# thu-ml/zhusuan

Hardware: NVIDIA H100
Metric: leapfrog-steps*chains/sec (higher is better)
Workload: dtype f32

## Files before the change

zhusuan_b200/csrc/hmc_dense_res.cu:

```cuda
#include "hmc_dense_epilogue.cuh"

namespace {

struct ResEpi {
  const __half* __restrict__ hi_cur; const __half* __restrict__ lo_cur;
  __half* __restrict__ hi_nxt; __half* __restrict__ lo_nxt;
  const __half* __restrict__ hi_cur_s; const __half* __restrict__ lo_cur_s;
  __half* __restrict__ hi_nxt_s; __half* __restrict__ lo_nxt_s;
  const float* __restrict__ p_in; float* __restrict__ p_out;
  float* __restrict__ lp_part; float* __restrict__ k_part;
  int64_t chains; int D;
  float sq, inv_sq, acc_scale;
  float rescale;
};

template <int MODE, int NEXT, int DC, bool SPARE>
__device__ __forceinline__ void epilogue_planes(const ResEpi& a, uint32_t trow, int n, bool n_ok,
                                                int64_t c0, int64_t part_row, int lane, float s2,
                                                float eps_over_m_sq, float inv_m, float b_n,
                                                float mu_n, float& qmax) {
  constexpr int NCOL = BN;
  const uint32_t D = DC ? (uint32_t)DC : (uint32_t)a.D;
  const int64_t chains = a.chains;
  const bool warp_n_ok = __all_sync(0xffffffffu, n_ok);
  const bool fast_tile = warp_n_ok && (c0 + NCOL <= chains);
  const int64_t off_t = c0 * (int64_t)D + n;
  const float* __restrict__ pin0 = a.p_in + off_t;
  float* __restrict__ po0 = a.p_out + off_t;
  const unsigned short* __restrict__ hc0 =
      reinterpret_cast<const unsigned short*>(a.hi_cur) + off_t;
  const unsigned short* __restrict__ lc0 =
      reinterpret_cast<const unsigned short*>(a.lo_cur) + off_t;
  __half* __restrict__ hn0 = NEXT ? a.hi_nxt + off_t : nullptr;
  __half* __restrict__ ln0 = NEXT ? a.lo_nxt + off_t : nullptr;
  __half* __restrict__ hs0 = SPARE ? a.hi_nxt_s + off_t : nullptr;
  __half* __restrict__ ls0 = SPARE ? a.lo_nxt_s + off_t : nullptr;

  auto element = [&](float acc, float p, uint32_t hl, float& pn, float& lpv, float& kv,
                     float& Qn) {
    const float Q = __half2float(__ushort_as_half((unsigned short)(hl & 0xFFFFu))) +
                    __half2float(__ushort_as_half((unsigned short)(hl >> 16)));
    const float g = b_n - a.acc_scale * acc;
    pn = fmaf(s2, g, p);
    if (MODE >= 1) lpv = (Q * a.inv_sq - mu_n) * g;
    if (MODE >= 2) kv = pn * pn * inv_m;
    if (NEXT) Qn = fmaf(eps_over_m_sq, pn, Q);
  };

  if (fast_tile) {
    auto load = [&](float* pe, uint32_t* he, int c) {
      const size_t cb = (size_t)c * D;
#pragma unroll
      for (int j = 0; j < 16; ++j) {
        pe[j] = __ldcg(pin0 + cb + (uint32_t)j * D);
        const uint32_t h = __ldcg(hc0 + cb + (uint32_t)j * D);
        const uint32_t l = __ldcg(lc0 + cb + (uint32_t)j * D);
        he[j] = h | (l << 16);
      }
    };
    float ss_a = 0.f, ss_b = 0.f;
    auto compute = [&](const uint32_t* v, const float* pe, const uint32_t* he, int c, float& ss) {
      const size_t cb = (size_t)c * D;
      float lpv[MODE >= 1 ? 16 : 1], kv[MODE >= 2 ? 16 : 1];
#pragma unroll
      for (int j = 0; j < 16; j += 2) {
        float pn[2], lp1[2] = {0.f, 0.f}, k1[2] = {0.f, 0.f}, Qn[2] = {0.f, 0.f};
#pragma unroll
        for (int t = 0; t < 2; ++t) {
          element(__uint_as_float(v[j + t]), pe[j + t], he[j + t], pn[t], lp1[t], k1[t], Qn[t]);
          po0[cb + (uint32_t)(j + t) * D] = pn[t];
          if (MODE >= 1) lpv[j + t] = lp1[t];
          if (MODE >= 2) kv[j + t] = k1[t];
          if (NEXT && !SPARE) ss = fmaf(Qn[t], Qn[t], ss);
          if (SPARE) qmax = fmaxf(qmax, fabsf(Qn[t]));
        }
        if (NEXT) {
          const __half2 h2 = __floats2half2_rn(Qn[0], Qn[1]);
          const float2 hf = __half22float2(h2);
          const __half2 l2 = __floats2half2_rn(Qn[0] - hf.x, Qn[1] - hf.y);
          hn0[cb + (uint32_t)j * D] = __low2half(h2);
          hn0[cb + (uint32_t)(j + 1) * D] = __high2half(h2);
          ln0[cb + (uint32_t)j * D] = __low2half(l2);
          ln0[cb + (uint32_t)(j + 1) * D] = __high2half(l2);
        }
        if (SPARE) {
          const float x0 = Qn[0] * a.rescale, x1 = Qn[1] * a.rescale;
          const __half2 h2 = __floats2half2_rn(x0, x1);
          const float2 hf = __half22float2(h2);
          const __half2 l2 = __floats2half2_rn(x0 - hf.x, x1 - hf.y);
          hs0[cb + (uint32_t)j * D] = __low2half(h2);
          hs0[cb + (uint32_t)(j + 1) * D] = __high2half(h2);
          ls0[cb + (uint32_t)j * D] = __low2half(l2);
          ls0[cb + (uint32_t)(j + 1) * D] = __high2half(l2);
        }
      }
      if (MODE >= 1) {
        const float sum = warp_transpose_sum16(lpv, lane);
        if (lane < 16) a.lp_part[part_row + c0 + c + lane] = sum;
      }
      if (MODE >= 2) {
        const float sum = warp_transpose_sum16(kv, lane);
        if (lane < 16) a.k_part[part_row + c0 + c + lane] = sum;
      }
    };
    float pa[16], pb[16];
    uint32_t ha[16], hb[16], va[16], vb[16];
    load(pa, ha, 0);
#pragma unroll 1
    for (int c = 0; c < NCOL; c += 32) {
      load(pb, hb, c + 16);
      acc_ld16(trow + 4u * (uint32_t)c, va);
      compute(va, pa, ha, c, ss_a);
      if (c + 32 < NCOL) load(pa, ha, c + 32);
      acc_ld16(trow + 4u * (uint32_t)(c + 16), vb);
      compute(vb, pb, hb, c + 16, ss_b);
    }
    if (NEXT && !SPARE) {
      const float norm = sqrtf(ss_a + ss_b) * (1.f + 0x1p-10f);
      qmax = fmaxf(qmax, norm == norm ? norm : INFINITY);
    }
  } else {
#pragma unroll 1
    for (int c = 0; c < NCOL; c += 16) {
      uint32_t v[16];
      acc_ld16(trow + 4u * (uint32_t)c, v);
      const int64_t cbase = c0 + c;
      if (cbase < chains) {
        const size_t cb = (size_t)c * D;
        float lpv[MODE >= 1 ? 16 : 1], kv[MODE >= 2 ? 16 : 1];
#pragma unroll
        for (int j = 0; j < 16; ++j) {
          const bool ok = n_ok && cbase + j < chains;
          float p = 0.f;
          uint32_t hl = 0u;
          if (ok) {
            p = __ldcg(pin0 + cb + (uint32_t)j * D);
            hl = (uint32_t)__ldcg(hc0 + cb + (uint32_t)j * D) |
                 ((uint32_t)__ldcg(lc0 + cb + (uint32_t)j * D) << 16);
          }
          float pn, lp1 = 0.f, k1 = 0.f, Qn = 0.f;
          element(__uint_as_float(v[j]), p, hl, pn, lp1, k1, Qn);
          const __half hh = __float2half_rn(Qn);
          const __half ll = __float2half_rn(Qn - __half2float(hh));
          if (NEXT && ok) qmax = fmaxf(qmax, fabsf(Qn));
          if (MODE >= 1) lpv[j] = ok ? lp1 : 0.f;
          if (MODE >= 2) kv[j] = ok ? k1 : 0.f;
          if (ok) {
            po0[cb + (uint32_t)j * D] = pn;
            if (NEXT) {
              hn0[cb + (uint32_t)j * D] = hh;
              ln0[cb + (uint32_t)j * D] = ll;
            }
            if (SPARE) {
              const float x = Qn * a.rescale;
              const __half hs = __float2half_rn(x);
              hs0[cb + (uint32_t)j * D] = hs;
              ls0[cb + (uint32_t)j * D] = __float2half_rn(x - __half2float(hs));
            }
          }
        }
        if (MODE >= 1) {
          const float sum = warp_transpose_sum16(lpv, lane);
          if (lane < 16 && cbase + lane < chains) a.lp_part[part_row + cbase + lane] = sum;
        }
        if (MODE >= 2) {
          const float sum = warp_transpose_sum16(kv, lane);
          if (lane < 16 && cbase + lane < chains) a.k_part[part_row + cbase + lane] = sum;
        }
      }
    }
  }
}


__device__ __forceinline__ int& producer_spare_in() {
  __shared__ int spare_in;
  return spare_in;
}

template <int MODE, int NEXT, int DC, int CX, int CY>
struct ResW {
  static constexpr int KIND = 1, RB = 64, MNA = 0, MNB = 0;
  static constexpr int CLUSTER = CX * CY;
  static constexpr int KE = RB / 2;
  static constexpr uint32_t TX = Cfg<RB>::STAGE;
  CUtensorMap m_phi, m_plo, m_qhi, m_qlo, m_shi, m_slo;
  ResEpi ea;
  const float* bvec; const float* mu; const float* mass; const float* state;
  float* scales;
  float p_scale;
  int n_blk, D_rt, pass;
  struct EpiState { float qmax = 0.f; };

  __device__ __forceinline__ int D() const { return DC ? DC : D_rt; }
  __host__ __device__ __forceinline__ int64_t units() const {
    return ((ea.chains + BN - 1) / BN) * (int64_t)n_blk;
  }
  __device__ __forceinline__ void tile(int64_t u, int& nb, int64_t& cb) const {
    const uint64_t cu = (uint64_t)u / CLUSTER;
    const int r = (int)((uint64_t)u % CLUSTER);
    const uint32_t nbx = (uint32_t)(n_blk / CX);
    nb = (int)(cu % nbx) * CX + r % CX;
    cb = (int64_t)(cu / nbx) * CY + r / CX;
  }
  __device__ __forceinline__ void kb_range(int64_t, int& kb0, int& kb1) const {
    kb0 = 0;
    kb1 = D() / KE;
  }
  __device__ __forceinline__ void prefetch() const {
    tma_prefetch_desc(&m_phi); tma_prefetch_desc(&m_plo);
    tma_prefetch_desc(&m_qhi); tma_prefetch_desc(&m_qlo);
    tma_prefetch_desc(&m_shi); tma_prefetch_desc(&m_slo);
    producer_spare_in() = plane_spare_in(scales, pass);
  }
  __device__ __forceinline__ void load(int64_t u, int kb, uint32_t sa, uint32_t fb) const {
    using C = Cfg<RB>;
    int nb;
    int64_t cb;
    tile(u, nb, cb);
    const int n0 = nb * BM;
    const int c0 = (int)cb * BN;
    const bool s = producer_spare_in() != 0;
    const CUtensorMap* qh = s ? &m_shi : &m_qhi;
    const CUtensorMap* ql = s ? &m_slo : &m_qlo;
    const int r = (int)(u % CLUSTER), rx = r % CX, ry = r / CX;
    if constexpr (CY == 1) {
      tma_load_2d(sa, &m_phi, fb, kb * KE, n0);
      tma_load_2d(sa + C::A_TILE, &m_plo, fb, kb * KE, n0);
    } else {
      constexpr int rows = BM / CY;
      uint16_t mask = 0;
#pragma unroll
      for (int y = 0; y < CY; ++y) mask |= (uint16_t)(1u << (y * CX + rx));
      const uint32_t o = (uint32_t)(ry * rows * RB);
      tma_load_2d_mc(sa + o, &m_phi, fb, kb * KE, n0 + ry * rows, mask);
      tma_load_2d_mc(sa + C::A_TILE + o, &m_plo, fb, kb * KE, n0 + ry * rows, mask);
    }
    if constexpr (CX == 1) {
      tma_load_2d(sa + 2 * C::A_TILE, qh, fb, kb * KE, c0);
      tma_load_2d(sa + 2 * C::A_TILE + C::B_TILE, ql, fb, kb * KE, c0);
    } else {
      constexpr int rows = BN / CX;
      const uint16_t mask = (uint16_t)(((1u << CX) - 1u) << (ry * CX));
      const uint32_t o = (uint32_t)(rx * rows * RB);
      tma_load_2d_mc(sa + 2 * C::A_TILE + o, qh, fb, kb * KE, c0 + rx * rows, mask);
      tma_load_2d_mc(sa + 2 * C::A_TILE + C::B_TILE + o, ql, fb, kb * KE, c0 + rx * rows, mask);
    }
  }
  __device__ __forceinline__ float sq_alt(float eps, float sq) const {
    return next_plane_scale(scales, pass, eps, mul(eps, p_scale), sq);
  }
  __device__ __forceinline__ void epilogue(int64_t u, uint32_t trow, int quarter, int lane,
                                           EpiState& st) const {
    int nb;
    int64_t cb;
    tile(u, nb, cb);
    const int n = nb * BM + quarter * 32 + lane;
    const int64_t c0 = cb * BN;
    const bool n_ok = n < D();
    const float eps = state[ZSB_ST_EPS_USED];
    const float s2 = mul(eps, p_scale);
    const bool spare_in = plane_spare_in(scales, pass);
    const float sq = plane_scale_in(scales, pass);
    const float m_n = n_ok ? mass[n] : 1.f;
    const float eps_over_m_sq = mul(fdiv(eps, m_n), sq);
    const float inv_m = fdiv(1.f, m_n);
    const float b_n = (n_ok && bvec) ? bvec[n] : 0.f;
    const float mu_n = (n_ok && mu) ? mu[n] : 0.f;
    const int64_t part_row = (int64_t)(nb * 4 + quarter) * ea.chains;
    ResEpi a = ea;
    if (spare_in) {
      a.hi_cur = ea.hi_cur_s;
      a.lo_cur = ea.lo_cur_s;
    }
    a.sq = sq;
    a.inv_sq = fdiv(1.f, sq);
    a.acc_scale = 1.f / (scales[3] * sq);
    a.rescale = NEXT ? sq_alt(eps, sq) * a.inv_sq : 1.f;
    if (a.rescale == 1.f)
      epilogue_planes<MODE, NEXT, DC, false>(a, trow, n, n_ok, c0, part_row, lane, s2,
                                             eps_over_m_sq, inv_m, b_n, mu_n, st.qmax);
    else
      epilogue_planes<MODE, NEXT, DC, true>(a, trow, n, n_ok, c0, part_row, lane, s2,
                                            eps_over_m_sq, inv_m, b_n, mu_n, st.qmax);
  }
  __device__ __forceinline__ void epi_finish(EpiState& st, int quarter, int lane) const {
    if (!NEXT) return;
    const float sq = plane_scale_in(scales, pass);
    const float alt = sq_alt(state[ZSB_ST_EPS_USED], sq);
    publish_plane_scale(scales, pass, sq, alt, st.qmax * (1.f / sq),
                        alt != sq && !(st.qmax < kHalfOverflow), quarter, lane);
  }
};

constexpr int RES_CX = 2, RES_CY = 1;

template <int DC, int CX, int CY>
int res_pass(const CUtensorMap& phi, const CUtensorMap& plo, const CUtensorMap& qhi,
             const CUtensorMap& qlo, const CUtensorMap& shi, const CUtensorMap& slo,
             const ResEpi& ea, const float* bvec, const float* mu, const float* mass,
             const float* state, float* scales, int pass, float p_scale, int n_blk, int D,
             int mode, cudaStream_t st) {
  if (mode == 1) {
    const ResW<1, 1, DC, CX, CY> w{phi, plo, qhi, qlo, shi, slo, ea, bvec, mu, mass, state,
                                   scales, p_scale, n_blk, D, pass};
    return tc_launch(w, st, "hmc_dense_resident");
  }
  if (mode == 0) {
    const ResW<0, 1, DC, CX, CY> w{phi, plo, qhi, qlo, shi, slo, ea, bvec, mu, mass, state,
                                   scales, p_scale, n_blk, D, pass};
    return tc_launch(w, st, "hmc_dense_resident");
  }
  const ResW<2, 0, DC, CX, CY> w{phi, plo, qhi, qlo, shi, slo, ea, bvec, mu, mass, state, scales,
                                 p_scale, n_blk, D, pass};
  return tc_launch(w, st, "hmc_dense_resident");
}

template <int DC>
int res_pass(bool cluster, const CUtensorMap& phi, const CUtensorMap& plo, const CUtensorMap& qhi,
             const CUtensorMap& qlo, const CUtensorMap& shi, const CUtensorMap& slo,
             const ResEpi& ea, const float* bvec, const float* mu, const float* mass,
             const float* state, float* scales, int pass, float p_scale, int n_blk, int D,
             int mode, cudaStream_t st) {
// ... 35 lines not shown
          const uint32_t lw[4] = {l[u].x, l[u].y, l[u].z, l[u].w};
          float o[8];
#pragma unroll
          for (int k = 0; k < 4; ++k) {
            const float2 hf = __half22float2(*reinterpret_cast<const __half2*>(&hw[k]));
            const float2 lf = __half22float2(*reinterpret_cast<const __half2*>(&lw[k]));
            o[2 * k] = (hf.x + lf.x) * inv_sq;
            o[2 * k + 1] = (hf.y + lf.y) * inv_sq;
          }
          qr[2 * i] = make_float4(o[0], o[1], o[2], o[3]);
          qr[2 * i + 1] = make_float4(o[4], o[5], o[6], o[7]);
        }
      }
    }
  }
}

}

int zsb_dense_res_h16_launch(void* planes0, void* planes1, void* spare0, void* spare1,
                             const float* p0, float* pw,
                             const void* P_h16, const void* P_l16, float* scales,
                             const float* bvec, const float* mu, const float* mass,
                             const float* state, float* lp0_part, float* lp1_part, float* k_part,
                             int64_t chains, int D, int L, cudaStream_t st) {
  if (D % 64 != 0 || D < 64 || L < 1 || chains <= 0 || chains >= (1LL << 31)) {
    zsb_set_error("dense_res: needs D %% 64 == 0, n_leapfrogs >= 1");
    return ZSB_ERR_INVALID;
  }
  if (planes0 == planes1 || !spare0 || !spare1 || spare0 == spare1) {
    zsb_set_error("dense_res: planes1, spare0 and spare1 must be separate work buffers");
    return ZSB_ERR_INVALID;
  }
  const int n_blk = (D + BM - 1) / BM;
  const int64_t c_blk = (chains + BN - 1) / BN;
  const bool cluster = n_blk % RES_CX == 0 && c_blk % RES_CY == 0;
  const uint32_t p_box = cluster ? BM / RES_CY : BM, q_box = cluster ? BN / RES_CX : BN;
  CUtensorMap phi, plo, qhi[2], qlo[2], shi[2], slo[2];
  int rc;
  constexpr int RB = ResW<0, 1, 0, 1, 1>::RB;
  if ((rc = make_map(&phi, P_h16, (uint64_t)D, (uint64_t)D, p_box, RB, 1))) return rc;
  if ((rc = make_map(&plo, P_l16, (uint64_t)D, (uint64_t)D, p_box, RB, 1))) return rc;
  __half* pl[2] = {reinterpret_cast<__half*>(planes0), reinterpret_cast<__half*>(planes1)};
  __half* sp[2] = {reinterpret_cast<__half*>(spare0), reinterpret_cast<__half*>(spare1)};
  const int64_t plane = chains * (int64_t)D;
  for (int b = 0; b < 2; ++b) {
    if ((rc = make_map(&qhi[b], pl[b], (uint64_t)chains, (uint64_t)D, q_box, RB, 1))) return rc;
    if ((rc = make_map(&qlo[b], pl[b] + plane, (uint64_t)chains, (uint64_t)D, q_box, RB, 1)))
      return rc;
    if ((rc = make_map(&shi[b], sp[b], (uint64_t)chains, (uint64_t)D, q_box, RB, 1))) return rc;
    if ((rc = make_map(&slo[b], sp[b] + plane, (uint64_t)chains, (uint64_t)D, q_box, RB, 1)))
      return rc;
  }
  for (int i = 0; i <= L; ++i) {
    const bool last = i == L;
    const int buf = i & 1;
    const ResEpi ea{pl[buf], pl[buf] + plane, pl[buf ^ 1], pl[buf ^ 1] + plane,
                    sp[buf], sp[buf] + plane, sp[buf ^ 1], sp[buf ^ 1] + plane,
                    i == 0 ? p0 : pw, pw, i == 0 ? lp0_part : lp1_part, k_part, chains, D,
                    1.f, 1.f, 1.f, 1.f};
    const int mode = last ? 2 : (i == 0 ? 1 : 0);
    const float p_scale = (i > 0 && !last) ? 1.f : 0.5f;
    rc = (D == 1024)
             ? res_pass<1024>(cluster, phi, plo, qhi[buf], qlo[buf], shi[buf], slo[buf], ea, bvec,
                              mu, mass, state, scales, i, p_scale, n_blk, D, mode, st)
             : res_pass<0>(cluster, phi, plo, qhi[buf], qlo[buf], shi[buf], slo[buf], ea, bvec, mu,
                           mass, state, scales, i, p_scale, n_blk, D, mode, st);
    if (rc != ZSB_OK) return rc;
  }
  return ZSB_OK;
}

#ifdef ZSB_PASS_PROFILE
// ... 23 lines not shown
```

zhusuan_b200/csrc/tc_common.cuh:

```cuda
#pragma once
#include "common.cuh"
#include <cuda.h>
#include <cuda_fp16.h>

namespace {

constexpr int BM = 128;
constexpr int BN = 128;
constexpr int NUM_EPI_WARPS = 4;
constexpr int PRODUCER_WARP = 4;
constexpr int EPI_WARP0 = 5;
constexpr int NUM_THREADS = 32 * (EPI_WARP0 + NUM_EPI_WARPS);
constexpr int ACC_LD = BN + 4;
constexpr int ACC_BYTES = BM * ACC_LD * 4;
constexpr unsigned long long WAIT_TIMEOUT_NS = 2000000000ULL;

enum PassProfSlot {
  PROF_MMA_TOTAL,
  PROF_MMA_FULL,
  PROF_MMA_TEMPTY,
  PROF_MMA_STORE,
  PROF_PROD_EMPTY,
  PROF_EPI_TFULL,
  PROF_EPI_UNIT,
  PROF_UNITS,
  PASS_PROF_SLOTS
};
constexpr int PASS_PROF_CTAS = 1024;
#ifdef ZSB_PASS_PROFILE
constexpr bool kPassProfile = true;
__device__ unsigned long long g_pass_prof[PASS_PROF_CTAS * PASS_PROF_SLOTS];
#else
constexpr bool kPassProfile = false;
#endif
__device__ __forceinline__ long long prof_clock() {
  if constexpr (kPassProfile) return clock64();
  return 0;
}
__device__ __forceinline__ void prof_add(int slot, long long v) {
#ifdef ZSB_PASS_PROFILE
  if (blockIdx.x < PASS_PROF_CTAS)
    atomicAdd(&g_pass_prof[blockIdx.x * PASS_PROF_SLOTS + slot], (unsigned long long)v);
#endif
}

template <int RB>
struct Cfg {
  static constexpr int A_TILE = BM * RB;
  static constexpr int B_TILE = BN * RB;
  static constexpr int STAGE = 2 * A_TILE + 2 * B_TILE;
  static constexpr int STAGES = RB == 128 ? 2 : 5;
  static constexpr int ALIGN = RB == 128 ? 1024 : 512;
  static constexpr int SMEM = STAGES * STAGE + ACC_BYTES + 128 + ALIGN;
  static_assert(SMEM <= 227 * 1024, "operand ring exceeds shared memory");
};

__device__ __forceinline__ uint32_t smem_u32(const void* p) {
  return (uint32_t)__cvta_generic_to_shared(p);
}
__device__ __forceinline__ void mbar_init(uint32_t bar, uint32_t count) {
  asm volatile("mbarrier.init.shared::cta.b64 [%0], %1;" ::"r"(bar), "r"(count) : "memory");
}
__device__ __forceinline__ void mbar_expect_tx(uint32_t bar, uint32_t bytes) {
  asm volatile("mbarrier.arrive.expect_tx.shared::cta.b64 _, [%0], %1;" ::"r"(bar), "r"(bytes)
               : "memory");
}
__device__ __forceinline__ void mbar_arrive(uint32_t bar) {
  asm volatile("mbarrier.arrive.shared::cta.b64 _, [%0];" ::"r"(bar) : "memory");
}
__device__ __forceinline__ bool mbar_try_wait(uint32_t bar, uint32_t parity) {
  uint32_t ok;
  asm volatile(
      "{\n\t.reg .pred P1;\n\t"
      "mbarrier.try_wait.parity.shared::cta.b64 P1, [%1], %2;\n\t"
      "selp.b32 %0, 1, 0, P1;\n\t}"
      : "=r"(ok)
      : "r"(bar), "r"(parity)
      : "memory");
  return ok != 0;
}
__device__ __forceinline__ unsigned long long global_ns() {
  unsigned long long t;
  asm volatile("mov.u64 %0, %%globaltimer;" : "=l"(t));
  return t;
}
__device__ __forceinline__ void mbar_wait(uint32_t bar, uint32_t parity) {
  if (mbar_try_wait(bar, parity)) return;
// ... 45 lines not shown
    d |= (uint64_t)1 << 62;
  } else {
    d |= (uint64_t)1 << 16;
    d |= (uint64_t)((8 * RB) >> 4) << 32;
    d |= (uint64_t)(RB == 128 ? 1 : 2) << 62;
  }
  return d;
}
__device__ __forceinline__ void wgmma_fence() {
  asm volatile("wgmma.fence.sync.aligned;" ::: "memory");
}
__device__ __forceinline__ void wgmma_commit() {
  asm volatile("wgmma.commit_group.sync.aligned;" ::: "memory");
}
template <int N>
__device__ __forceinline__ void wgmma_wait() {
  asm volatile("wgmma.wait_group.sync.aligned %0;" ::"n"(N) : "memory");
}
__device__ __forceinline__ void wgmma_tf32(float (&d)[64], uint64_t da, uint64_t db) {
  asm volatile(
      "{\n\t.reg .pred p;\n\tsetp.ne.b32 p, 1, 0;\n\t"
      "wgmma.mma_async.sync.aligned.m64n128k8.f32.tf32.tf32 {%0, %1, %2, %3, %4, %5, %6, %7, %8, %9, %10, %11, %12, %13, %14, %15, %16, %17, %18, %19, %20, %21, %22, %23, %24, %25, %26, %27, %28, %29, %30, %31, %32, %33, %34, %35, %36, %37, %38, %39, %40, %41, %42, %43, %44, %45, %46, %47, %48, %49, %50, %51, %52, %53, %54, %55, %56, %57, %58, %59, %60, %61, %62, %63}, %64, %65, p, 1, 1;\n\t}"
      : "+f"(d[0]), "+f"(d[1]), "+f"(d[2]), "+f"(d[3]), "+f"(d[4]), "+f"(d[5]), "+f"(d[6]), "+f"(d[7]), "+f"(d[8]), "+f"(d[9]), "+f"(d[10]), "+f"(d[11]), "+f"(d[12]), "+f"(d[13]), "+f"(d[14]), "+f"(d[15]), "+f"(d[16]), "+f"(d[17]), "+f"(d[18]), "+f"(d[19]), "+f"(d[20]), "+f"(d[21]), "+f"(d[22]), "+f"(d[23]), "+f"(d[24]), "+f"(d[25]), "+f"(d[26]), "+f"(d[27]), "+f"(d[28]), "+f"(d[29]), "+f"(d[30]), "+f"(d[31]), "+f"(d[32]), "+f"(d[33]), "+f"(d[34]), "+f"(d[35]), "+f"(d[36]), "+f"(d[37]), "+f"(d[38]), "+f"(d[39]), "+f"(d[40]), "+f"(d[41]), "+f"(d[42]), "+f"(d[43]), "+f"(d[44]), "+f"(d[45]), "+f"(d[46]), "+f"(d[47]), "+f"(d[48]), "+f"(d[49]), "+f"(d[50]), "+f"(d[51]), "+f"(d[52]), "+f"(d[53]), "+f"(d[54]), "+f"(d[55]), "+f"(d[56]), "+f"(d[57]), "+f"(d[58]), "+f"(d[59]), "+f"(d[60]), "+f"(d[61]), "+f"(d[62]), "+f"(d[63])
      : "l"(da), "l"(db));
}
template <int TA, int TB>
__device__ __forceinline__ void wgmma_f16(float (&d)[64], uint64_t da, uint64_t db) {
  asm volatile(
      "{\n\t.reg .pred p;\n\tsetp.ne.b32 p, 1, 0;\n\t"
      "wgmma.mma_async.sync.aligned.m64n128k16.f32.f16.f16 {%0, %1, %2, %3, %4, %5, %6, %7, %8, %9, %10, %11, %12, %13, %14, %15, %16, %17, %18, %19, %20, %21, %22, %23, %24, %25, %26, %27, %28, %29, %30, %31, %32, %33, %34, %35, %36, %37, %38, %39, %40, %41, %42, %43, %44, %45, %46, %47, %48, %49, %50, %51, %52, %53, %54, %55, %56, %57, %58, %59, %60, %61, %62, %63}, %64, %65, p, 1, 1, %66, %67;\n\t}"
      : "+f"(d[0]), "+f"(d[1]), "+f"(d[2]), "+f"(d[3]), "+f"(d[4]), "+f"(d[5]), "+f"(d[6]), "+f"(d[7]), "+f"(d[8]), "+f"(d[9]), "+f"(d[10]), "+f"(d[11]), "+f"(d[12]), "+f"(d[13]), "+f"(d[14]), "+f"(d[15]), "+f"(d[16]), "+f"(d[17]), "+f"(d[18]), "+f"(d[19]), "+f"(d[20]), "+f"(d[21]), "+f"(d[22]), "+f"(d[23]), "+f"(d[24]), "+f"(d[25]), "+f"(d[26]), "+f"(d[27]), "+f"(d[28]), "+f"(d[29]), "+f"(d[30]), "+f"(d[31]), "+f"(d[32]), "+f"(d[33]), "+f"(d[34]), "+f"(d[35]), "+f"(d[36]), "+f"(d[37]), "+f"(d[38]), "+f"(d[39]), "+f"(d[40]), "+f"(d[41]), "+f"(d[42]), "+f"(d[43]), "+f"(d[44]), "+f"(d[45]), "+f"(d[46]), "+f"(d[47]), "+f"(d[48]), "+f"(d[49]), "+f"(d[50]), "+f"(d[51]), "+f"(d[52]), "+f"(d[53]), "+f"(d[54]), "+f"(d[55]), "+f"(d[56]), "+f"(d[57]), "+f"(d[58]), "+f"(d[59]), "+f"(d[60]), "+f"(d[61]), "+f"(d[62]), "+f"(d[63])
      : "l"(da), "l"(db), "n"(TA), "n"(TB));
}

__device__ __forceinline__ void acc_ld16(uint32_t addr, uint32_t v[16]) {
#pragma unroll
  for (int i = 0; i < 4; ++i)
    asm volatile("ld.shared.v4.b32 {%0, %1, %2, %3}, [%4];"
                 : "=r"(v[4 * i]), "=r"(v[4 * i + 1]), "=r"(v[4 * i + 2]), "=r"(v[4 * i + 3])
                 : "r"(addr + 16u * i));
}

__device__ __forceinline__ float warp_transpose_sum16(float v[16], int lane) {
#pragma unroll
  for (int i = 0; i < 16; ++i) v[i] += __shfl_xor_sync(0xffffffffu, v[i], 16);
#pragma unroll
  for (int o = 8, cnt = 16; o >= 1; o >>= 1, cnt >>= 1) {
    const bool upper = (lane & o) != 0;
#pragma unroll
    for (int i = 0; i < cnt / 2; ++i) {
      const float keep = upper ? v[i + cnt / 2] : v[i];
      const float send = upper ? v[i] : v[i + cnt / 2];
      v[i] = keep + __shfl_xor_sync(0xffffffffu, send, o);
    }
  }
  return v[0];
}

__device__ __forceinline__ float pow2_plane_scale(float m) {
  int e = 0;
  if (m > 0.f) frexpf(m, &e);
  return ldexpf(1.f, 12 - e);
}
__device__ __forceinline__ float finite_absmax(float m, float x) {
  const float a = fabsf(x);
  return (a <= 3.0e38f) ? fmaxf(m, a) : m;
}
__device__ __forceinline__ void store_hilo(__half* p, int64_t lo, float x) {
  const __half h = __float2half_rn(x);
  p[0] = h;
  p[lo] = __float2half_rn(x - __half2float(h));
}
__device__ __forceinline__ void fold_amax(float* scale, float m, int lane) {
  m = warp_max(m);
  if (lane == 0 && m > 0.f) atomicMax(reinterpret_cast<unsigned int*>(scale) + 2, __float_as_uint(m));
}

template <int KIND, int RB, int MNA, int MNB, int ZLO = 0>
__device__ __forceinline__ void mma_kblock(float (&d)[2][64], uint32_t sa) {
  using C = Cfg<RB>;
#pragma unroll
  for (int k = 0; k < RB / 32; ++k) {
    const uint32_t bo = MNB ? (uint32_t)k * 2048u : (uint32_t)k * 32u;
    const uint64_t b_hi = gmma_desc<MNB, RB>(sa + 2 * C::A_TILE + bo);
    const uint64_t b_lo = gmma_desc<MNB, RB>(sa + 2 * C::A_TILE + C::B_TILE + bo);
#pragma unroll
    for (int mh = 0; mh < 2; ++mh) {
      const uint32_t ao = MNA ? (uint32_t)mh * 8192u + (uint32_t)k * 2048u
                              : (uint32_t)(mh * 64 * RB) + (uint32_t)k * 32u;
      const uint64_t a_hi = gmma_desc<MNA, RB>(sa + ao);
      const uint64_t a_lo = gmma_desc<MNA, RB>(sa + C::A_TILE + ao);
      if (KIND == 0) {
        wgmma_tf32(d[mh], a_lo, b_hi);
        wgmma_tf32(d[mh], a_hi, b_lo);
        wgmma_tf32(d[mh], a_hi, b_hi);
      } else {
        if (!(ZLO & 1)) wgmma_f16<MNA, MNB>(d[mh], a_lo, b_hi);
        if (!(ZLO & 2)) wgmma_f16<MNA, MNB>(d[mh], a_hi, b_lo);
        wgmma_f16<MNA, MNB>(d[mh], a_hi, b_hi);
      }
    }
  }
}

template <class W, class = void>
struct ClusterOf {
  static constexpr int value = 1;
};
template <class W>
struct ClusterOf<W, decltype((void)W::CLUSTER)> {
  static constexpr int value = W::CLUSTER;
};

template <class W, class = void>
struct ZloOf {
  static constexpr int value = 0;
};
template <class W>
struct ZloOf<W, decltype((void)W::ZLO)> {
  static constexpr int value = W::ZLO;
};

template <class W>
__global__ void __launch_bounds__(NUM_THREADS, 1) tc_pipeline_kernel(const __grid_constant__ W w) {
  using C = Cfg<W::RB>;
  constexpr int CS = ClusterOf<W>::value;
  extern __shared__ uint8_t smem_raw[];
  const uint32_t smem_base = (smem_u32(smem_raw) + (C::ALIGN - 1)) & ~(uint32_t)(C::ALIGN - 1);
  const uint32_t acc_base = smem_base + C::STAGES * C::STAGE;
  const uint32_t bars = acc_base + ACC_BYTES;
  const uint32_t full_bar = bars;
  const uint32_t empty_bar = bars + 8 * C::STAGES;
  const uint32_t tfull_bar = bars + 16 * C::STAGES;
  const uint32_t tempty_bar = tfull_bar + 8;

  const int warp = __shfl_sync(0xffffffffu, (int)(threadIdx.x >> 5), 0);
  const int lane = threadIdx.x & 31;
  const int64_t n_units = w.units();

  if (threadIdx.x == 0) {
    for (int s = 0; s < C::STAGES; ++s) {
      mbar_init(full_bar + 8 * s, 1);
      mbar_init(empty_bar + 8 * s, CS);
    }
    mbar_init(tfull_bar, 128);
    mbar_init(tempty_bar, 32 * NUM_EPI_WARPS);
    asm volatile("fence.mbarrier_init.release.cluster;" ::: "memory");
  }
  if constexpr (CS > 1)
    cluster_sync();
  else
    __syncthreads();
  auto release = [&](int s) {
    if constexpr (CS > 1) {
#pragma unroll
      for (int r = 0; r < CS; ++r) mbar_arrive_cluster(empty_bar + 8 * s, (uint32_t)r);
    } else {
      mbar_arrive(empty_bar + 8 * s);
    }
  };

  if (warp < 4) {
    const int tid = threadIdx.x;
    float d[2][64];
    int stage = 0;
    uint32_t phase = 0, acc_phase = 0;
    const long long t_begin = prof_clock();
    long long t_full = 0, t_tempty = 0, t_store = 0, units = 0;
    for (int64_t u = blockIdx.x; u < n_units; u += gridDim.x) {
      int kb0, kb1;
      w.kb_range(u, kb0, kb1);
#pragma unroll
      for (int mh = 0; mh < 2; ++mh)
#pragma unroll
        for (int i = 0; i < 64; ++i) d[mh][i] = 0.f;
      int prev = -1;
      for (int kb = kb0; kb < kb1; ++kb) {
        const uint32_t sa = smem_base + stage * C::STAGE;
        const long long t0 = prof_clock();
        mbar_spin(full_bar + 8 * stage, phase);
        t_full += prof_clock() - t0;
        wgmma_fence();
        mma_kblock<W::KIND, W::RB, W::MNA, W::MNB, ZloOf<W>::value>(d, sa);
        wgmma_commit();
        wgmma_wait<1>();
        if (prev >= 0 && tid == 0) release(prev);
        prev = stage;
        if (++stage == C::STAGES) { stage = 0; phase ^= 1; }
      }
      wgmma_wait<0>();
      if (prev >= 0 && tid == 0) release(prev);
      const long long t1 = prof_clock();
      mbar_wait(tempty_bar, acc_phase ^ 1);
      const long long t2 = prof_clock();
      t_tempty += t2 - t1;
      const int row = 16 * (tid >> 5) + ((tid & 31) >> 2);
      const int col = 2 * (tid & 3);
#pragma unroll
      for (int mh = 0; mh < 2; ++mh)
#pragma unroll
        for (int j = 0; j < 16; ++j) {
          const uint32_t a0 = acc_base + (uint32_t)(((64 * mh + row) * ACC_LD + 8 * j + col) * 4);
          asm volatile("st.shared.v2.f32 [%0], {%1, %2};" ::"r"(a0), "f"(d[mh][4 * j]),
                       "f"(d[mh][4 * j + 1]) : "memory");
          asm volatile("st.shared.v2.f32 [%0], {%1, %2};" ::"r"(a0 + 8u * ACC_LD * 4u),
                       "f"(d[mh][4 * j + 2]), "f"(d[mh][4 * j + 3]) : "memory");
        }
      mbar_arrive(tfull_bar);
      acc_phase ^= 1;
      t_store += prof_clock() - t2;
      ++units;
    }
    if (kPassProfile && tid == 0) {
      prof_add(PROF_MMA_TOTAL, prof_clock() - t_begin);
      prof_add(PROF_MMA_FULL, t_full);
      prof_add(PROF_MMA_TEMPTY, t_tempty);
      prof_add(PROF_MMA_STORE, t_store);
      prof_add(PROF_UNITS, units);
    }
  } else if (warp == PRODUCER_WARP) {
    if (lane == 0) {
      w.prefetch();
      int stage = 0;
      uint32_t phase = 0;
      long long t_empty = 0;
      for (int64_t u = blockIdx.x; u < n_units; u += gridDim.x) {
        int kb0, kb1;
        w.kb_range(u, kb0, kb1);
        for (int kb = kb0; kb < kb1; ++kb) {
          const long long t0 = prof_clock();
          mbar_wait(empty_bar + 8 * stage, phase ^ 1);
          t_empty += prof_clock() - t0;
          const uint32_t fb = full_bar + 8 * stage;
          mbar_expect_tx(fb, W::TX);
          w.load(u, kb, smem_base + stage * C::STAGE, fb);
          if (++stage == C::STAGES) { stage = 0; phase ^= 1; }
        }
      }
      if (kPassProfile) prof_add(PROF_PROD_EMPTY, t_empty);
    }
  } else {
    const int quarter = warp - EPI_WARP0;
    const uint32_t trow = acc_base + (uint32_t)((quarter * 32 + lane) * ACC_LD * 4);
    typename W::EpiState st;
    uint32_t acc_phase = 0;
    long long t_tfull = 0, t_unit = 0;
    for (int64_t u = blockIdx.x; u < n_units; u += gridDim.x) {
      const long long t0 = prof_clock();
      mbar_wait(tfull_bar, acc_phase);
      const long long t1 = prof_clock();
      w.epilogue(u, trow, quarter, lane, st);
      __syncwarp();
      mbar_arrive(tempty_bar);
      acc_phase ^= 1;
      t_tfull += t1 - t0;
      t_unit += prof_clock() - t1;
    }
    if (kPassProfile && quarter == 0 && lane == 0) {
      prof_add(PROF_EPI_TFULL, t_tfull);
      prof_add(PROF_EPI_UNIT, t_unit);
    }
    w.epi_finish(st, quarter, lane);
  }
  if constexpr (CS > 1) cluster_sync();
}

template <class W>
int tc_launch(const W& w, cudaStream_t st, const char* what) {
  constexpr int CS = ClusterOf<W>::value;
  static const cudaError_t attr = cudaFuncSetAttribute(
      tc_pipeline_kernel<W>, cudaFuncAttributeMaxDynamicSharedMemorySize, Cfg<W::RB>::SMEM);
  if (attr != cudaSuccess) {
    zsb_set_error("%s: cudaFuncSetAttribute: %s", what, cudaGetErrorString(attr));
    return ZSB_ERR_CUDA;
  }
  if constexpr (CS > 1) {
    const int64_t units = w.units();
    if (units < 1 || units % CS != 0) {
      zsb_set_error("%s: %lld units do not tile by clusters of %d", what, (long long)units, CS);
      return ZSB_ERR_INVALID;
    }
    cudaLaunchAttribute cl[1];
    cl[0].id = cudaLaunchAttributeClusterDimension;
    cl[0].val.clusterDim.x = CS;
    cl[0].val.clusterDim.y = 1;
    cl[0].val.clusterDim.z = 1;
    cudaLaunchConfig_t cfg = {};
    cfg.blockDim = dim3(NUM_THREADS);
    cfg.dynamicSmemBytes = Cfg<W::RB>::SMEM;
    cfg.stream = st;
    cfg.attrs = cl;
    cfg.numAttrs = 1;
    static int max_clusters = 0;
    if (max_clusters < 1) {
      cfg.gridDim = dim3(CS);
      const cudaError_t e =
          cudaOccupancyMaxActiveClusters(&max_clusters, tc_pipeline_kernel<W>, &cfg);
      if (e != cudaSuccess || max_clusters < 1) {
        zsb_set_error("%s: no cluster of %d CTAs fits (%s)", what, CS, cudaGetErrorString(e));
        max_clusters = 0;
        return ZSB_ERR_CUDA;
      }
    }
    int64_t grid = (int64_t)max_clusters * CS;
    if (grid > units) grid = units;
    cfg.gridDim = dim3((unsigned)grid);
    const cudaError_t e = cudaLaunchKernelEx(&cfg, tc_pipeline_kernel<W>, w);
    if (e != cudaSuccess) {
      zsb_set_error("%s: cudaLaunchKernelEx: %s", what, cudaGetErrorString(e));
      return ZSB_ERR_CUDA;
    }
    return zsb_check_launch(what);
  } else {
    int dev = 0, sms = ZSB_NUM_SMS;
    cudaGetDevice(&dev);
    cudaDeviceGetAttribute(&sms, cudaDevAttrMultiProcessorCount, dev);
    int64_t grid = w.units();
    if (grid > sms) grid = sms;
    if (grid < 1) grid = 1;
    tc_pipeline_kernel<W><<<(unsigned)grid, NUM_THREADS, Cfg<W::RB>::SMEM, st>>>(w);
    return zsb_check_launch(what);
  }
}

typedef CUresult (*EncodeTiledFn)(CUtensorMap*, CUtensorMapDataType, cuuint32_t, void*,
                                  const cuuint64_t*, const cuuint64_t*, const cuuint32_t*,
                                  const cuuint32_t*, CUtensorMapInterleave, CUtensorMapSwizzle,
                                  CUtensorMapL2promotion, CUtensorMapFloatOOBfill);

EncodeTiledFn get_encode_fn() {
  static EncodeTiledFn fn = nullptr;
  if (!fn) {
    void* p = nullptr;
    cudaDriverEntryPointQueryResult qres;
    if (cudaGetDriverEntryPoint("cuTensorMapEncodeTiled", &p, cudaEnableDefault, &qres) !=
            cudaSuccess || qres != cudaDriverEntryPointSuccess)
      return nullptr;
    fn = (EncodeTiledFn)p;
  }
  return fn;
}

int make_map(CUtensorMap* map, const void* base, uint64_t rows, uint64_t cols, uint32_t box_rows,
             int rb, int half_elems = 0) {
  EncodeTiledFn enc = get_encode_fn();
  if (!enc) {
    zsb_set_error("tc: cuTensorMapEncodeTiled unavailable");
    return ZSB_ERR_CUDA;
  }
  const int esz = half_elems ? 2 : 4;
  cuuint64_t dims[2] = {cols, rows};
  cuuint64_t strides[1] = {cols * esz};
  cuuint32_t box[2] = {(cuuint32_t)(rb / esz), box_rows};
// ... 15 lines not shown
```

Before: 72.56 million.

## Widen residual GEMM tile to N=160 with warp-specialized register reallocation

The residual kernel now uses a 64x160 wgmma tile (new m64n160k16 instruction). It reorganizes the CTA into 384 threads with setmaxnreg so MMA and epilogue warps get more registers while the producer warps give theirs up. The pipeline stage count is now derived from the shared-memory budget. The aim is more accumulator reuse per loaded A tile and fewer units to schedule. Smaller edits swap fdiv/sqrtf for custom division and approximate-sqrt helpers, fold the norm twice for wide tiles, and use 32-bit tile index math, at the cost of register pressure and possible epilogue spills.

```diff
diff --git a/zhusuan_b200/csrc/hmc_dense_res.cu b/zhusuan_b200/csrc/hmc_dense_res.cu
--- a/zhusuan_b200/csrc/hmc_dense_res.cu
+++ b/zhusuan_b200/csrc/hmc_dense_res.cu
@@ -1,6 +1,23 @@
 #include "hmc_dense_epilogue.cuh"
 
 namespace {
+
+__device__ __forceinline__ float div_rn(float a, float b) {
+  const double ad = (double)a, bd = (double)b;
+  double r;
+  asm("rcp.approx.ftz.f64 %0, %1;" : "=d"(r) : "d"(bd));
+  if (a == 0.f || b == 0.f || !(fabsf(a) <= 3.4028235e38f) || !(fabsf(b) <= 3.4028235e38f))
+    return __double2float_rn(ad * r);
+  r = fma(r, fma(-bd, r, 1.0), r);
+  r = fma(r, fma(-bd, r, 1.0), r);
+  const double q = ad * r;
+  return __double2float_rn(fma(r, fma(-bd, q, ad), q));
+}
+__device__ __forceinline__ float sqrt_up(float x) {
+  float y;
+  asm("sqrt.approx.f32 %0, %1;" : "=f"(y) : "f"(x));
+  return y * (1.f + 0x1p-20f);
+}
 
 struct ResEpi {
   const __half* __restrict__ hi_cur; const __half* __restrict__ lo_cur;
@@ -14,12 +31,12 @@
   float rescale;
 };
 
-template <int MODE, int NEXT, int DC, bool SPARE>
+template <int MODE, int NEXT, int DC, bool SPARE, int NCOL>
 __device__ __forceinline__ void epilogue_planes(const ResEpi& a, uint32_t trow, int n, bool n_ok,
                                                 int64_t c0, int64_t part_row, int lane, float s2,
                                                 float eps_over_m_sq, float inv_m, float b_n,
                                                 float mu_n, float& qmax) {
-  constexpr int NCOL = BN;
+  static_assert(NCOL % 32 == 0 && NCOL <= 256, "the 32-column software pipeline");
   const uint32_t D = DC ? (uint32_t)DC : (uint32_t)a.D;
   const int64_t chains = a.chains;
   const bool warp_n_ok = __all_sync(0xffffffffu, n_ok);
@@ -59,6 +76,11 @@
       }
     };
     float ss_a = 0.f, ss_b = 0.f;
+    auto fold_norm = [&]() {
+      const float norm = sqrt_up(ss_a + ss_b) * (1.f + 0x1p-10f);
+      qmax = fmaxf(qmax, norm == norm ? norm : INFINITY);
+      ss_a = ss_b = 0.f;
+    };
     auto compute = [&](const uint32_t* v, const float* pe, const uint32_t* he, int c, float& ss) {
       const size_t cb = (size_t)c * D;
       float lpv[MODE >= 1 ? 16 : 1], kv[MODE >= 2 ? 16 : 1];
@@ -95,11 +117,11 @@
         }
       }
       if (MODE >= 1) {
-        const float sum = warp_transpose_sum16(lpv, lane);
+        const float sum = warp_transpose_sum16<true>(lpv, lane);
         if (lane < 16) a.lp_part[part_row + c0 + c + lane] = sum;
       }
       if (MODE >= 2) {
-        const float sum = warp_transpose_sum16(kv, lane);
+        const float sum = warp_transpose_sum16<true>(kv, lane);
         if (lane < 16) a.k_part[part_row + c0 + c + lane] = sum;
       }
     };
@@ -114,11 +136,9 @@
       if (c + 32 < NCOL) load(pa, ha, c + 32);
       acc_ld16(trow + 4u * (uint32_t)(c + 16), vb);
       compute(vb, pb, hb, c + 16, ss_b);
-    }
-    if (NEXT && !SPARE) {
-      const float norm = sqrtf(ss_a + ss_b) * (1.f + 0x1p-10f);
-      qmax = fmaxf(qmax, norm == norm ? norm : INFINITY);
-    }
+      if (NEXT && !SPARE && NCOL > 128 && c + 32 == 128) fold_norm();
+    }
+    if (NEXT && !SPARE) fold_norm();
   } else {
 #pragma unroll 1
     for (int c = 0; c < NCOL; c += 16) {
@@ -160,11 +180,11 @@
           }
         }
         if (MODE >= 1) {
-          const float sum = warp_transpose_sum16(lpv, lane);
+          const float sum = warp_transpose_sum16<true>(lpv, lane);
           if (lane < 16 && cbase + lane < chains) a.lp_part[part_row + cbase + lane] = sum;
         }
         if (MODE >= 2) {
-          const float sum = warp_transpose_sum16(kv, lane);
+          const float sum = warp_transpose_sum16<true>(kv, lane);
           if (lane < 16 && cbase + lane < chains) a.k_part[part_row + cbase + lane] = sum;
         }
       }
@@ -180,10 +200,12 @@
 
 template <int MODE, int NEXT, int DC, int CX, int CY>
 struct ResW {
-  static constexpr int KIND = 1, RB = 64, MNA = 0, MNB = 0;
+  static constexpr int KIND = 1, RB = 64, MNA = 0, MNB = 0, BN = 160;
+  static constexpr bool SPLIT_REGS = true;
   static constexpr int CLUSTER = CX * CY;
   static constexpr int KE = RB / 2;
-  static constexpr uint32_t TX = Cfg<RB>::STAGE;
+  using C = Cfg<RB, BN>;
+  static constexpr uint32_t TX = C::STAGE;
   CUtensorMap m_phi, m_plo, m_qhi, m_qlo, m_shi, m_slo;
   ResEpi ea;
   const float* bvec; const float* mu; const float* mass; const float* state;
@@ -197,8 +219,8 @@
     return ((ea.chains + BN - 1) / BN) * (int64_t)n_blk;
   }
   __device__ __forceinline__ void tile(int64_t u, int& nb, int64_t& cb) const {
-    const uint64_t cu = (uint64_t)u / CLUSTER;
-    const int r = (int)((uint64_t)u % CLUSTER);
+    const uint32_t cu = (uint32_t)u / CLUSTER;
+    const int r = (int)((uint32_t)u % CLUSTER);
     const uint32_t nbx = (uint32_t)(n_blk / CX);
     nb = (int)(cu % nbx) * CX + r % CX;
     cb = (int64_t)(cu / nbx) * CY + r / CX;
@@ -214,7 +236,6 @@
     producer_spare_in() = plane_spare_in(scales, pass);
   }
   __device__ __forceinline__ void load(int64_t u, int kb, uint32_t sa, uint32_t fb) const {
-    using C = Cfg<RB>;
     int nb;
     int64_t cb;
     tile(u, nb, cb);
@@ -263,8 +284,8 @@
     const bool spare_in = plane_spare_in(scales, pass);
     const float sq = plane_scale_in(scales, pass);
     const float m_n = n_ok ? mass[n] : 1.f;
-    const float eps_over_m_sq = mul(fdiv(eps, m_n), sq);
-    const float inv_m = fdiv(1.f, m_n);
+    const float eps_over_m_sq = mul(div_rn(eps, m_n), sq);
+    const float inv_m = div_rn(1.f, m_n);
     const float b_n = (n_ok && bvec) ? bvec[n] : 0.f;
     const float mu_n = (n_ok && mu) ? mu[n] : 0.f;
     const int64_t part_row = (int64_t)(nb * 4 + quarter) * ea.chains;
@@ -274,21 +295,21 @@
       a.lo_cur = ea.lo_cur_s;
     }
     a.sq = sq;
-    a.inv_sq = fdiv(1.f, sq);
-    a.acc_scale = 1.f / (scales[3] * sq);
+    a.inv_sq = div_rn(1.f, sq);
+    a.acc_scale = div_rn(1.f, scales[3] * sq);
     a.rescale = NEXT ? sq_alt(eps, sq) * a.inv_sq : 1.f;
     if (a.rescale == 1.f)
-      epilogue_planes<MODE, NEXT, DC, false>(a, trow, n, n_ok, c0, part_row, lane, s2,
+      epilogue_planes<MODE, NEXT, DC, false, BN>(a, trow, n, n_ok, c0, part_row, lane, s2,
                                              eps_over_m_sq, inv_m, b_n, mu_n, st.qmax);
     else
-      epilogue_planes<MODE, NEXT, DC, true>(a, trow, n, n_ok, c0, part_row, lane, s2,
+      epilogue_planes<MODE, NEXT, DC, true, BN>(a, trow, n, n_ok, c0, part_row, lane, s2,
                                             eps_over_m_sq, inv_m, b_n, mu_n, st.qmax);
   }
   __device__ __forceinline__ void epi_finish(EpiState& st, int quarter, int lane) const {
     if (!NEXT) return;
     const float sq = plane_scale_in(scales, pass);
     const float alt = sq_alt(state[ZSB_ST_EPS_USED], sq);
-    publish_plane_scale(scales, pass, sq, alt, st.qmax * (1.f / sq),
+    publish_plane_scale(scales, pass, sq, alt, st.qmax * div_rn(1.f, sq),
                         alt != sq && !(st.qmax < kHalfOverflow), quarter, lane);
   }
 };
@@ -390,13 +411,17 @@
     zsb_set_error("dense_res: planes1, spare0 and spare1 must be separate work buffers");
     return ZSB_ERR_INVALID;
   }
+  constexpr int RB = ResW<0, 1, 0, 1, 1>::RB, RN = ResW<0, 1, 0, 1, 1>::BN;
   const int n_blk = (D + BM - 1) / BM;
-  const int64_t c_blk = (chains + BN - 1) / BN;
+  const int64_t c_blk = (chains + RN - 1) / RN;
+  if (c_blk * n_blk >= (1LL << 32)) {
+    zsb_set_error("dense_res: %lld units exceed 2^32", (long long)(c_blk * n_blk));
+    return ZSB_ERR_INVALID;
+  }
   const bool cluster = n_blk % RES_CX == 0 && c_blk % RES_CY == 0;
-  const uint32_t p_box = cluster ? BM / RES_CY : BM, q_box = cluster ? BN / RES_CX : BN;
+  const uint32_t p_box = cluster ? BM / RES_CY : BM, q_box = cluster ? RN / RES_CX : RN;
   CUtensorMap phi, plo, qhi[2], qlo[2], shi[2], slo[2];
   int rc;
-  constexpr int RB = ResW<0, 1, 0, 1, 1>::RB;
   if ((rc = make_map(&phi, P_h16, (uint64_t)D, (uint64_t)D, p_box, RB, 1))) return rc;
   if ((rc = make_map(&plo, P_l16, (uint64_t)D, (uint64_t)D, p_box, RB, 1))) return rc;
   __half* pl[2] = {reinterpret_cast<__half*>(planes0), reinterpret_cast<__half*>(planes1)};
diff --git a/zhusuan_b200/csrc/tc_common.cuh b/zhusuan_b200/csrc/tc_common.cuh
--- a/zhusuan_b200/csrc/tc_common.cuh
+++ b/zhusuan_b200/csrc/tc_common.cuh
@@ -12,7 +12,7 @@
 constexpr int EPI_WARP0 = 5;
 constexpr int NUM_THREADS = 32 * (EPI_WARP0 + NUM_EPI_WARPS);
 constexpr int ACC_LD = BN + 4;
-constexpr int ACC_BYTES = BM * ACC_LD * 4;
+constexpr int SMEM_MAX = 227 * 1024;
 constexpr unsigned long long WAIT_TIMEOUT_NS = 2000000000ULL;
 
 enum PassProfSlot {
@@ -44,15 +44,18 @@
 #endif
 }
 
-template <int RB>
+template <int RB, int TN = BN>
 struct Cfg {
   static constexpr int A_TILE = BM * RB;
-  static constexpr int B_TILE = BN * RB;
+  static constexpr int B_TILE = TN * RB;
   static constexpr int STAGE = 2 * A_TILE + 2 * B_TILE;
-  static constexpr int STAGES = RB == 128 ? 2 : 5;
+  static constexpr int ACC_LD = TN + 4;
+  static constexpr int ACC_BYTES = BM * ACC_LD * 4;
   static constexpr int ALIGN = RB == 128 ? 1024 : 512;
+  static constexpr int STAGES = (SMEM_MAX - ACC_BYTES - 128 - ALIGN) / STAGE;
   static constexpr int SMEM = STAGES * STAGE + ACC_BYTES + 128 + ALIGN;
-  static_assert(SMEM <= 227 * 1024, "operand ring exceeds shared memory");
+  static_assert(STAGES >= 2 && SMEM <= SMEM_MAX, "operand ring exceeds shared memory");
+  static_assert(B_TILE % ALIGN == 0 && STAGE % ALIGN == 0, "operand tiles break the swizzle");
 };
 
 __device__ __forceinline__ uint32_t smem_u32(const void* p) {
@@ -164,6 +167,22 @@
       : "+f"(d[0]), "+f"(d[1]), "+f"(d[2]), "+f"(d[3]), "+f"(d[4]), "+f"(d[5]), "+f"(d[6]), "+f"(d[7]), "+f"(d[8]), "+f"(d[9]), "+f"(d[10]), "+f"(d[11]), "+f"(d[12]), "+f"(d[13]), "+f"(d[14]), "+f"(d[15]), "+f"(d[16]), "+f"(d[17]), "+f"(d[18]), "+f"(d[19]), "+f"(d[20]), "+f"(d[21]), "+f"(d[22]), "+f"(d[23]), "+f"(d[24]), "+f"(d[25]), "+f"(d[26]), "+f"(d[27]), "+f"(d[28]), "+f"(d[29]), "+f"(d[30]), "+f"(d[31]), "+f"(d[32]), "+f"(d[33]), "+f"(d[34]), "+f"(d[35]), "+f"(d[36]), "+f"(d[37]), "+f"(d[38]), "+f"(d[39]), "+f"(d[40]), "+f"(d[41]), "+f"(d[42]), "+f"(d[43]), "+f"(d[44]), "+f"(d[45]), "+f"(d[46]), "+f"(d[47]), "+f"(d[48]), "+f"(d[49]), "+f"(d[50]), "+f"(d[51]), "+f"(d[52]), "+f"(d[53]), "+f"(d[54]), "+f"(d[55]), "+f"(d[56]), "+f"(d[57]), "+f"(d[58]), "+f"(d[59]), "+f"(d[60]), "+f"(d[61]), "+f"(d[62]), "+f"(d[63])
       : "l"(da), "l"(db), "n"(TA), "n"(TB));
 }
+template <int TA, int TB>
+__device__ __forceinline__ void wgmma_f16(float (&d)[80], uint64_t da, uint64_t db) {
+  asm volatile(
+      "{\n\t.reg .pred p;\n\tsetp.ne.b32 p, 1, 0;\n\t"
+      "wgmma.mma_async.sync.aligned.m64n160k16.f32.f16.f16 {%0, %1, %2, %3, %4, %5, %6, %7, %8, %9, %10, %11, %12, %13, %14, %15, %16, %17, %18, %19, %20, %21, %22, %23, %24, %25, %26, %27, %28, %29, %30, %31, %32, %33, %34, %35, %36, %37, %38, %39, %40, %41, %42, %43, %44, %45, %46, %47, %48, %49, %50, %51, %52, %53, %54, %55, %56, %57, %58, %59, %60, %61, %62, %63, %64, %65, %66, %67, %68, %69, %70, %71, %72, %73, %74, %75, %76, %77, %78, %79}, %80, %81, p, 1, 1, %82, %83;\n\t}"
+      : "+f"(d[0]), "+f"(d[1]), "+f"(d[2]), "+f"(d[3]), "+f"(d[4]), "+f"(d[5]), "+f"(d[6]), "+f"(d[7]), "+f"(d[8]), "+f"(d[9]), "+f"(d[10]), "+f"(d[11]), "+f"(d[12]), "+f"(d[13]), "+f"(d[14]), "+f"(d[15]), "+f"(d[16]), "+f"(d[17]), "+f"(d[18]), "+f"(d[19]), "+f"(d[20]), "+f"(d[21]), "+f"(d[22]), "+f"(d[23]), "+f"(d[24]), "+f"(d[25]), "+f"(d[26]), "+f"(d[27]), "+f"(d[28]), "+f"(d[29]), "+f"(d[30]), "+f"(d[31]), "+f"(d[32]), "+f"(d[33]), "+f"(d[34]), "+f"(d[35]), "+f"(d[36]), "+f"(d[37]), "+f"(d[38]), "+f"(d[39]), "+f"(d[40]), "+f"(d[41]), "+f"(d[42]), "+f"(d[43]), "+f"(d[44]), "+f"(d[45]), "+f"(d[46]), "+f"(d[47]), "+f"(d[48]), "+f"(d[49]), "+f"(d[50]), "+f"(d[51]), "+f"(d[52]), "+f"(d[53]), "+f"(d[54]), "+f"(d[55]), "+f"(d[56]), "+f"(d[57]), "+f"(d[58]), "+f"(d[59]), "+f"(d[60]), "+f"(d[61]), "+f"(d[62]), "+f"(d[63]), "+f"(d[64]), "+f"(d[65]), "+f"(d[66]), "+f"(d[67]), "+f"(d[68]), "+f"(d[69]), "+f"(d[70]), "+f"(d[71]), "+f"(d[72]), "+f"(d[73]), "+f"(d[74]), "+f"(d[75]), "+f"(d[76]), "+f"(d[77]), "+f"(d[78]), "+f"(d[79])
+      : "l"(da), "l"(db), "n"(TA), "n"(TB));
+}
+template <int R>
+__device__ __forceinline__ void setmaxnreg_inc() {
+  asm volatile("setmaxnreg.inc.sync.aligned.u32 %0;" ::"n"(R));
+}
+template <int R>
+__device__ __forceinline__ void setmaxnreg_dec() {
+  asm volatile("setmaxnreg.dec.sync.aligned.u32 %0;" ::"n"(R));
+}
 
 __device__ __forceinline__ void acc_ld16(uint32_t addr, uint32_t v[16]) {
 #pragma unroll
@@ -173,6 +192,7 @@
                  : "r"(addr + 16u * i));
 }
 
+template <bool IN_REGS = false>
 __device__ __forceinline__ float warp_transpose_sum16(float v[16], int lane) {
 #pragma unroll
   for (int i = 0; i < 16; ++i) v[i] += __shfl_xor_sync(0xffffffffu, v[i], 16);
@@ -180,10 +200,12 @@
   for (int o = 8, cnt = 16; o >= 1; o >>= 1, cnt >>= 1) {
     const bool upper = (lane & o) != 0;
 #pragma unroll
-    for (int i = 0; i < cnt / 2; ++i) {
-      const float keep = upper ? v[i + cnt / 2] : v[i];
-      const float send = upper ? v[i] : v[i + cnt / 2];
-      v[i] = keep + __shfl_xor_sync(0xffffffffu, send, o);
+    for (int i = 0; i < (IN_REGS ? 8 : cnt / 2); ++i) {
+      if (!IN_REGS || i < cnt / 2) {
+        const float keep = upper ? v[i + cnt / 2] : v[i];
+        const float send = upper ? v[i] : v[i + cnt / 2];
+        v[i] = keep + __shfl_xor_sync(0xffffffffu, send, o);
+      }
     }
   }
   return v[0];
@@ -208,9 +230,10 @@
   if (lane == 0 && m > 0.f) atomicMax(reinterpret_cast<unsigned int*>(scale) + 2, __float_as_uint(m));
 }
 
-template <int KIND, int RB, int MNA, int MNB, int ZLO = 0>
-__device__ __forceinline__ void mma_kblock(float (&d)[2][64], uint32_t sa) {
-  using C = Cfg<RB>;
+template <int KIND, int RB, int MNA, int MNB, int ZLO = 0, int NA = 64>
+__device__ __forceinline__ void mma_kblock(float (&d)[2][NA], uint32_t sa) {
+  using C = Cfg<RB, 2 * NA>;
+  static_assert(NA == 64 || (KIND == 1 && MNB == 0), "wide units: fp16 K-major B only");
 #pragma unroll
   for (int k = 0; k < RB / 32; ++k) {
     const uint32_t bo = MNB ? (uint32_t)k * 2048u : (uint32_t)k * 32u;
@@ -222,7 +245,7 @@
                               : (uint32_t)(mh * 64 * RB) + (uint32_t)k * 32u;
       const uint64_t a_hi = gmma_desc<MNA, RB>(sa + ao);
       const uint64_t a_lo = gmma_desc<MNA, RB>(sa + C::A_TILE + ao);
-      if (KIND == 0) {
+      if constexpr (KIND == 0) {
         wgmma_tf32(d[mh], a_lo, b_hi);
         wgmma_tf32(d[mh], a_hi, b_lo);
         wgmma_tf32(d[mh], a_hi, b_hi);
@@ -253,14 +276,40 @@
   static constexpr int value = W::ZLO;
 };
 
+template <class W, class = void>
+struct BnOf {
+  static constexpr int value = BN;
+};
 template <class W>
-__global__ void __launch_bounds__(NUM_THREADS, 1) tc_pipeline_kernel(const __grid_constant__ W w) {
-  using C = Cfg<W::RB>;
+struct BnOf<W, decltype((void)W::BN)> {
+  static constexpr int value = W::BN;
+};
+
+template <class W, class = void>
+struct Roles {
+  static constexpr bool SPLIT = false;
+  static constexpr int THREADS = NUM_THREADS;
+  static constexpr int EPI0 = EPI_WARP0;
+};
+template <class W>
+struct Roles<W, decltype((void)W::SPLIT_REGS)> {
+  static constexpr bool SPLIT = W::SPLIT_REGS;
+  static constexpr int THREADS = SPLIT ? 384 : NUM_THREADS;
+  static constexpr int EPI0 = SPLIT ? 8 : EPI_WARP0;
+  static constexpr int MMA_REGS = 200, PRODUCER_REGS = 40, EPI_REGS = 256;
+};
+
+template <class W>
+__global__ void __launch_bounds__(Roles<W>::THREADS, 1)
+    tc_pipeline_kernel(const __grid_constant__ W w) {
+  constexpr int TN = BnOf<W>::value;
+  using C = Cfg<W::RB, TN>;
+  using R = Roles<W>;
   constexpr int CS = ClusterOf<W>::value;
   extern __shared__ uint8_t smem_raw[];
   const uint32_t smem_base = (smem_u32(smem_raw) + (C::ALIGN - 1)) & ~(uint32_t)(C::ALIGN - 1);
   const uint32_t acc_base = smem_base + C::STAGES * C::STAGE;
-  const uint32_t bars = acc_base + ACC_BYTES;
+  const uint32_t bars = acc_base + C::ACC_BYTES;
   const uint32_t full_bar = bars;
   const uint32_t empty_bar = bars + 8 * C::STAGES;
   const uint32_t tfull_bar = bars + 16 * C::STAGES;
@@ -293,8 +342,9 @@
   };
 
   if (warp < 4) {
+    if constexpr (R::SPLIT) setmaxnreg_inc<R::MMA_REGS>();
     const int tid = threadIdx.x;
-    float d[2][64];
+    float d[2][TN / 2];
     int stage = 0;
     uint32_t phase = 0, acc_phase = 0;
     const long long t_begin = prof_clock();
@@ -305,7 +355,7 @@
 #pragma unroll
       for (int mh = 0; mh < 2; ++mh)
 #pragma unroll
-        for (int i = 0; i < 64; ++i) d[mh][i] = 0.f;
+        for (int i = 0; i < TN / 2; ++i) d[mh][i] = 0.f;
       int prev = -1;
       for (int kb = kb0; kb < kb1; ++kb) {
         const uint32_t sa = smem_base + stage * C::STAGE;
@@ -313,7 +363,7 @@
         mbar_spin(full_bar + 8 * stage, phase);
         t_full += prof_clock() - t0;
         wgmma_fence();
-        mma_kblock<W::KIND, W::RB, W::MNA, W::MNB, ZloOf<W>::value>(d, sa);
+        mma_kblock<W::KIND, W::RB, W::MNA, W::MNB, ZloOf<W>::value, TN / 2>(d, sa);
         wgmma_commit();
         wgmma_wait<1>();
         if (prev >= 0 && tid == 0) release(prev);
@@ -331,11 +381,12 @@
 #pragma unroll
       for (int mh = 0; mh < 2; ++mh)
 #pragma unroll
-        for (int j = 0; j < 16; ++j) {
-          const uint32_t a0 = acc_base + (uint32_t)(((64 * mh + row) * ACC_LD + 8 * j + col) * 4);
+        for (int j = 0; j < TN / 8; ++j) {
+          const uint32_t a0 =
+              acc_base + (uint32_t)(((64 * mh + row) * C::ACC_LD + 8 * j + col) * 4);
           asm volatile("st.shared.v2.f32 [%0], {%1, %2};" ::"r"(a0), "f"(d[mh][4 * j]),
                        "f"(d[mh][4 * j + 1]) : "memory");
-          asm volatile("st.shared.v2.f32 [%0], {%1, %2};" ::"r"(a0 + 8u * ACC_LD * 4u),
+          asm volatile("st.shared.v2.f32 [%0], {%1, %2};" ::"r"(a0 + 8u * C::ACC_LD * 4u),
                        "f"(d[mh][4 * j + 2]), "f"(d[mh][4 * j + 3]) : "memory");
         }
       mbar_arrive(tfull_bar);
@@ -350,8 +401,9 @@
       prof_add(PROF_MMA_STORE, t_store);
       prof_add(PROF_UNITS, units);
     }
-  } else if (warp == PRODUCER_WARP) {
-    if (lane == 0) {
+  } else if (R::SPLIT ? warp < R::EPI0 : warp == PRODUCER_WARP) {
+    if constexpr (R::SPLIT) setmaxnreg_dec<R::PRODUCER_REGS>();
+    if ((!R::SPLIT || warp == PRODUCER_WARP) && lane == 0) {
       w.prefetch();
       int stage = 0;
       uint32_t phase = 0;
@@ -372,8 +424,9 @@
       if (kPassProfile) prof_add(PROF_PROD_EMPTY, t_empty);
     }
   } else {
-    const int quarter = warp - EPI_WARP0;
-    const uint32_t trow = acc_base + (uint32_t)((quarter * 32 + lane) * ACC_LD * 4);
+    if constexpr (R::SPLIT) setmaxnreg_inc<R::EPI_REGS>();
+    const int quarter = warp - R::EPI0;
+    const uint32_t trow = acc_base + (uint32_t)((quarter * 32 + lane) * C::ACC_LD * 4);
     typename W::EpiState st;
     uint32_t acc_phase = 0;
     long long t_tfull = 0, t_unit = 0;
@@ -400,11 +453,29 @@
 template <class W>
 int tc_launch(const W& w, cudaStream_t st, const char* what) {
   constexpr int CS = ClusterOf<W>::value;
+  constexpr int SMEM = Cfg<W::RB, BnOf<W>::value>::SMEM;
   static const cudaError_t attr = cudaFuncSetAttribute(
-      tc_pipeline_kernel<W>, cudaFuncAttributeMaxDynamicSharedMemorySize, Cfg<W::RB>::SMEM);
+      tc_pipeline_kernel<W>, cudaFuncAttributeMaxDynamicSharedMemorySize, SMEM);
   if (attr != cudaSuccess) {
     zsb_set_error("%s: cudaFuncSetAttribute: %s", what, cudaGetErrorString(attr));
     return ZSB_ERR_CUDA;
+  }
+  if constexpr (Roles<W>::SPLIT) {
+    using R = Roles<W>;
+    static int regs = -1;
+    if (regs < 0) {
+      cudaFuncAttributes fa;
+      if (cudaFuncGetAttributes(&fa, tc_pipeline_kernel<W>) != cudaSuccess) {
+        zsb_set_error("%s: cudaFuncGetAttributes failed", what);
+        return ZSB_ERR_CUDA;
+      }
+      regs = fa.numRegs;
+    }
+    if (regs * R::THREADS < 128 * (R::MMA_REGS + R::PRODUCER_REGS + R::EPI_REGS)) {
+      zsb_set_error("%s: %d registers per thread at launch do not cover the role budgets", what,
+                    regs);
+      return ZSB_ERR_INVALID;
+    }
   }
   if constexpr (CS > 1) {
     const int64_t units = w.units();
@@ -418,8 +489,8 @@
     cl[0].val.clusterDim.y = 1;
     cl[0].val.clusterDim.z = 1;
     cudaLaunchConfig_t cfg = {};
-    cfg.blockDim = dim3(NUM_THREADS);
-    cfg.dynamicSmemBytes = Cfg<W::RB>::SMEM;
+    cfg.blockDim = dim3(Roles<W>::THREADS);
+    cfg.dynamicSmemBytes = SMEM;
     cfg.stream = st;
     cfg.attrs = cl;
     cfg.numAttrs = 1;
@@ -450,7 +521,7 @@
     int64_t grid = w.units();
     if (grid > sms) grid = sms;
     if (grid < 1) grid = 1;
-    tc_pipeline_kernel<W><<<(unsigned)grid, NUM_THREADS, Cfg<W::RB>::SMEM, st>>>(w);
+    tc_pipeline_kernel<W><<<(unsigned)grid, Roles<W>::THREADS, SMEM, st>>>(w);
     return zsb_check_launch(what);
   }
 }
```

After: 76.31 million, median of 6. +5.2%, better.
